# sourmash-bio/sourmash

Hardware: AMD Instinct MI355X
Metric: Gbase/s sketched (k=31, scaled=1000) (higher is better)
Workload: dtype u64; 1 GPU; C2: sketch synthetic random DNA resident in HBM as ASCII, per GPU 1000 records of 10000000 bases (10000000000 bases, 10000001000 bytes with their separators), k=31 scaled=1000 seed=42; one step = k-mer kernel + radix sort + unique; records_per_gpu=1000, record_len=10000000, bases_per_gpu=10000000000, bytes_per_gpu=10000001000, ksize=31, scaled=1000, unique_hashes_rank0=9998668, unique_hashes_job=9998668, collectives=none (the exchange runs with --full)

## Files before the change

include/sourmash_amd.h:

```cpp
#ifndef SOURMASH_AMD_H_INCLUDED
#define SOURMASH_AMD_H_INCLUDED

#include <stdarg.h>
#include <stdbool.h>
#include <stdint.h>
#include <stdlib.h>

#ifdef __cplusplus
extern "C" {
#endif


enum {
  HASH_FUNCTIONS_MURMUR64_DNA = 1,
  HASH_FUNCTIONS_MURMUR64_PROTEIN = 2,
  HASH_FUNCTIONS_MURMUR64_DAYHOFF = 3,
  HASH_FUNCTIONS_MURMUR64_HP = 4,
};
typedef uint32_t HashFunctions;

enum {
  SOURMASH_ERROR_CODE_NO_ERROR = 0,
  SOURMASH_ERROR_CODE_PANIC = 1,
  SOURMASH_ERROR_CODE_INTERNAL = 2,
// ... 196 lines not shown
uint64_t smgpu_minhash_pending_bytes(const SourmashKmerMinHash *ptr);
uint64_t smgpu_signature_add_file(SourmashSignature *ptr, const char *path, uint64_t *n_records);
SourmashSignature **smgpu_sketch_files(const char *const *paths, uintptr_t n, const SourmashComputeParameters *params,
                                       uint32_t n_threads, uint64_t *total_bases);
uint64_t smgpu_minhash_add_file(SourmashKmerMinHash *ptr, const char *path, uint64_t *n_records);
uint64_t smgpu_gunzip_files(const char *const *paths, uintptr_t n, uint8_t *out, uint64_t capacity, uint64_t *lens, double *stats);
void smgpu_sigload_counters(uint64_t *out);
void smgpu_gunzip_counters(uint64_t *out);

uint64_t smgpu_sketch_workspace_bytes(uint64_t out_capacity);
uint64_t smgpu_sketch_dna_raw(const uint8_t *d_seq, uint64_t len, uint32_t ksize, uint64_t seed, uint64_t max_hash,
                              uint64_t *d_out, uint64_t out_capacity, uint64_t *d_result, void *d_workspace,
                              uint64_t workspace_bytes, void *stream);
uint64_t smgpu_sketch_records_workspace_bytes(uint64_t pair_capacity, uint64_t n_records);
uint64_t smgpu_sketch_records_raw(const uint8_t *d_seq, uint64_t len, const uint64_t *d_starts, uint64_t n_records,
                                  uint32_t ksize, uint64_t seed, uint64_t max_hash, uint64_t *d_hashes, uint64_t *d_abunds,
                                  uint64_t capacity, uint64_t *d_offsets, uint64_t *d_result, void *d_workspace,
                                  uint64_t workspace_bytes, void *stream);
void smgpu_sketch_records_kernel_raw(const uint8_t *d_seq, uint64_t len, uint32_t ksize, uint64_t seed, uint64_t max_hash,
                                     uint64_t *d_hashes, uint64_t *d_positions, uint64_t capacity, uint64_t *d_count, void *stream);
void smgpu_fastx_compact_raw(const uint8_t *d_raw, uint64_t len, int32_t fastq, uint8_t *d_carry, uint8_t *d_out, uint64_t *d_result,
                             uint64_t *d_record_starts, uint64_t record_capacity, int32_t last_piece, void *stream);
uint64_t smgpu_sigjson_text_pad(void);
void smgpu_sigjson_parse_raw(const uint8_t *d_text, uint64_t text_len, const uint64_t *docs, uint32_t n_docs, uint64_t keep_max,
                             void *spans_out, uint32_t *flags_out, uint64_t *d_values, uint64_t value_capacity, void *parsed_out,
                             uint64_t parsed_capacity, uint64_t *counts_out, void *stream);
SourmashSignature **smgpu_sketch_file_singleton(const char *path, const SourmashComputeParameters *params, uintptr_t *n);
void smgpu_sketch_dna_kernel_raw(const uint8_t *d_seq, uint64_t len, uint32_t ksize, uint64_t seed, uint64_t max_hash,
                                 uint64_t *d_out, uint64_t out_capacity, uint64_t *d_count, void *stream);
void smgpu_sketch_dna_kernel_grid_raw(const uint8_t *d_seq, uint64_t len, uint32_t ksize, uint64_t seed, uint64_t max_hash,
                                      uint64_t *d_out, uint64_t out_capacity, uint64_t *d_count, uint32_t grid, void *stream);
uint64_t smgpu_sort_unique_raw(uint64_t *d_keys, uint64_t n, uint64_t *d_out, uint64_t *d_n_out, void *d_workspace,
                               uint64_t workspace_bytes, void *stream);
uint64_t smgpu_sketch_residues_kernels_raw(const uint8_t *d_seq, uint64_t len, uint32_t k_aa, uint32_t hash_function, uint64_t seed,
                                           uint64_t max_hash, bool translate, uint8_t *d_aa, uint64_t aa_capacity, uint64_t *d_out,
                                           uint64_t out_capacity, uint64_t *d_count, void *stream);
void smgpu_synth_dna_raw(uint8_t *d_out, uint64_t start, uint64_t n, uint64_t seed, uint64_t record_len, void *stream);

void smgpu_compare_raw(const uint64_t *d_hashes, const uint64_t *d_offsets, uint32_t n, uint32_t row_lo,
                       uint32_t row_hi, uint32_t *d_common, double *d_jaccard, void *stream);
void smgpu_compare_blocks_raw(const uint64_t *d_hashes, const uint64_t *d_offsets, uint32_t n, uint32_t rb_first,
                              uint32_t rb_stride, uint32_t rb_count, uint32_t *d_common, void *stream);
void smgpu_symmetrize_raw(uint32_t *d_common, uint32_t n, void *stream);
void smgpu_jaccard_raw(const uint32_t *d_common, const uint64_t *d_offsets, uint32_t n, uint32_t row_lo,
                       uint32_t row_hi, double *d_jaccard, void *stream);
typedef struct SmgpuBitIndex SmgpuBitIndex;
SmgpuBitIndex *smgpu_bitindex_new(const uint64_t *d_hashes, const uint64_t *d_offsets, uint32_t n, void *stream);
SmgpuBitIndex *smgpu_bitindex_new_ex(const uint64_t *d_hashes, const uint64_t *d_offsets, uint32_t n, uint64_t total_hashes,
                                     uint32_t threshold, bool one_shot, void *stream);
void smgpu_bitindex_free(SmgpuBitIndex *ptr);
uint64_t smgpu_bitindex_universe(const SmgpuBitIndex *ptr);
uint32_t smgpu_bitindex_builder(const SmgpuBitIndex *ptr);
void smgpu_bitindex_stats(const SmgpuBitIndex *ptr, uint64_t *frequent_hashes, uint64_t *rare_pairs, uint32_t *threshold);
void smgpu_bitindex_compare_raw(const SmgpuBitIndex *ptr, uint32_t rb_first, uint32_t rb_stride, uint32_t rb_count,
                                uint32_t *d_common, void *stream);
void smgpu_bitindex_compare_upper_raw(const SmgpuBitIndex *ptr, uint32_t rb_first, uint32_t rb_stride, uint32_t rb_count,
                                      uint32_t *d_common, void *stream);
void smgpu_host_pow_f64(const double *x, const double *y, uintptr_t ny, double *out, uintptr_t n, uint32_t n_threads);
uintptr_t smgpu_first_invalid_dna_byte(const char *seq, uintptr_t len);
void smgpu_compare_all_pairs(const SourmashKmerMinHash *const *mhs, uintptr_t n, uint32_t *common_out,
                             double *jaccard_out);
void smgpu_compare_all_pairs_mixed(const SourmashKmerMinHash *const *mhs, uintptr_t n, const uint32_t *class_of,
                                   const uint64_t *class_max_hash, uintptr_t n_classes, uint32_t *common_out, uint64_t *sizes_out);
void smgpu_signatures_sketch_views(const SourmashSignature *const *sigs, uintptr_t n, const SourmashKmerMinHash **out_mhs,
                                   uint64_t *params);
void smgpu_minhashes_params(const SourmashKmerMinHash *const *mhs, uintptr_t n, uint64_t *params);
// ... 148 lines not shown
```

sourmash_amd/csrc/capi.cpp:

```cpp
#if defined(__SSE2__)
#include <emmintrin.h>
#endif
#include <hip/hip_runtime_api.h>
#include <stdio.h>
#include <string.h>
#include <chrono>
#include <cmath>
#include <fstream>
#include <memory>
#include <sstream>
#include <thread>
#include "../../include/sourmash_amd.h"
#include "collection.hpp"
#include <fcntl.h>
#include <sys/mman.h>
#include <sys/stat.h>
#include <unistd.h>
#include "device_ctx.hpp"
#include "hostxfer.hpp"
#include "pargz.hpp"
#include "ingest.hpp"
#include "sigload.hpp"
#include "murmur3.hpp"
#include "residues.hpp"
#include "signature_host.hpp"
#include "hll_host.hpp"
#include "nodegraph_host.hpp"

using namespace smg;

namespace {

thread_local uint32_t g_err_code = 0;
thread_local std::string g_err_msg;

void set_error(uint32_t code, const std::string& msg) { g_err_code = code; g_err_msg = msg; }

template <class R, class F>
R landing(F&& f) {
    try {
        return f();
    } catch (const Error& e) {
        set_error(e.code, e.what());
    } catch (const std::bad_alloc&) {
        set_error(E_PANIC, "sourmash panicked: out of memory");
    } catch (const std::exception& e) {
        set_error(E_PANIC, std::string("sourmash panicked: ") + e.what());
    } catch (...) {
        set_error(E_PANIC, "sourmash panicked: unknown exception");
    }
    return R{};
}
template <class F>
void landing_void(F&& f) {
    landing<int>([&]() { f(); return 0; });
}
// ... 707 lines not shown
            lens[i] = ms[i].out_len;
            at += ms[i].out_len;
        }
        hip_check(hipStreamSynchronize(st), "sync");
        if (stats) {
            const double v[10] = {(double)gs.survivors, (double)gs.candidates, (double)gs.runs, gs.scan_ms, gs.pass1_ms, gs.link_ms, gs.pass2_ms,
                                  gs.finish_ms, gs.total_ms, io_ms};
            for (int k = 0; k < 16; ++k) stats[k] = k < 10 ? v[k] : 0.0;
        }
        return at;
    });
}
void smgpu_sigload_counters(uint64_t* out) {
    if (!out) return;
    out[0] = sigload_counters().on_device.load();
    out[1] = sigload_counters().on_host.load();
}
void smgpu_gunzip_counters(uint64_t* out) {
    if (!out) return;
    out[0] = gunzip_counters().on_device.load();
    out[1] = gunzip_counters().refused.load();
}
uint64_t smgpu_minhash_add_file(SourmashKmerMinHash* p, const char* path, uint64_t* n_records) {
    return landing<uint64_t>([&]() -> uint64_t {
        if (!path) throw err_internal("null path");
        std::vector<KmerMinHash*> mhs{MH(p)};
        uint64_t recs = 0, bases = 0;
        sketch_file_into(mhs, path, &recs, &bases);
        if (n_records) *n_records = recs;
        return bases;
    });
}

uint64_t smgpu_sketch_workspace_bytes(uint64_t out_capacity) {
    return (uint64_t)out_capacity * 8 + sort_unique_temp_bytes(out_capacity) + 512;
}

uint64_t smgpu_sketch_dna_raw(const uint8_t* d_seq, uint64_t len, uint32_t ksize, uint64_t seed, uint64_t max_hash,
                              uint64_t* d_out, uint64_t cap, uint64_t* d_result, void* d_ws, uint64_t ws_bytes,
                              void* stream) {
    uint64_t ret = ~0ull;
    landing_void([&] {
        hipStream_t st = (hipStream_t)stream;
        if (ws_bytes < smgpu_sketch_workspace_bytes(cap)) throw err_internal("workspace too small (smgpu_sketch_workspace_bytes)");
        uint64_t* d_raw = (uint64_t*)d_ws;
        void* d_tmp = (char*)d_ws + ((cap * 8 + 255) / 256) * 256;
        const size_t tmp_bytes = (size_t)(ws_bytes - ((cap * 8 + 255) / 256) * 256);
        const uint64_t thr = max_hash ? max_hash : ~0ull;
        check_dna_ksize(ksize);
        hip_check(hipMemsetAsync(d_result, 0, 16, st), "memset");
        hip_check(sketch_dna_launch(d_seq, len, ksize, seed, thr, d_raw, (unsigned long long*)d_result, cap, st), "sketch_dna");
        unsigned long long kept = 0;
        hip_check(hipMemcpyAsync(&kept, d_result, 8, hipMemcpyDeviceToHost, st), "D2H");
        hip_check(hipStreamSynchronize(st), "sync");
        if (kept > cap)
            throw err_internal("output capacity too small: " + std::to_string(kept) + " kept hashes > capacity " + std::to_string(cap));
        int bits = 64;
        if (thr != ~0ull) { bits = 1; while (bits < 64 && (thr >> bits)) ++bits; }
        hip_check(sort_unique(d_raw, kept, d_out, nullptr, d_result + 1, d_tmp, tmp_bytes, bits, st), "sort_unique");
        unsigned long long nu = 0;
        hip_check(hipMemcpyAsync(&nu, d_result + 1, 8, hipMemcpyDeviceToHost, st), "D2H");
        hip_check(hipStreamSynchronize(st), "sync");
        ret = nu;
    });
    return ret;
}

uint64_t smgpu_sort_unique_raw(uint64_t* d_keys, uint64_t n, uint64_t* d_out, uint64_t* d_n_out, void* d_ws, uint64_t ws_bytes, void* stream) {
    uint64_t ret = ~0ull;
    landing_void([&] {
        hipStream_t st = (hipStream_t)stream;
        if (ws_bytes < sort_unique_temp_bytes(n)) throw err_internal("workspace too small (smgpu_sketch_workspace_bytes)");
        hip_check(sort_unique(d_keys, n, d_out, nullptr, d_n_out, d_ws, (size_t)ws_bytes, 64, st), "sort_unique");
        unsigned long long nu = 0;
        hip_check(hipMemcpyAsync(&nu, d_n_out, 8, hipMemcpyDeviceToHost, st), "D2H");
        hip_check(hipStreamSynchronize(st), "sync");
        ret = nu;
    });
    return ret;
}

void smgpu_sketch_dna_kernel_raw(const uint8_t* d_seq, uint64_t len, uint32_t ksize, uint64_t seed, uint64_t max_hash,
                                 uint64_t* d_out, uint64_t cap, uint64_t* d_count, void* stream) {
    landing_void([&] {
        check_dna_ksize(ksize);
        hip_check(sketch_dna_launch(d_seq, len, ksize, seed, max_hash ? max_hash : ~0ull, d_out,
                                    (unsigned long long*)d_count, cap, (hipStream_t)stream), "sketch_dna");
    });
}
void smgpu_sketch_dna_kernel_grid_raw(const uint8_t* d_seq, uint64_t len, uint32_t ksize, uint64_t seed, uint64_t max_hash,
                                      uint64_t* d_out, uint64_t cap, uint64_t* d_count, uint32_t grid, void* stream) {
    landing_void([&] {
        check_dna_ksize(ksize);
        if (grid > (1u << 20)) throw err_internal("grid: at most 1048576 workgroups");
// ... 2460 lines not shown
```

sourmash_amd/csrc/device_api.hpp:

```cpp
#pragma once
#include <hip/hip_runtime.h>
#include <stdint.h>
#include <stddef.h>
#include "find_core.hpp"

namespace smg {

hipError_t sketch_dna_launch(const uint8_t* d_seq, uint64_t len, uint32_t k, uint64_t seed, uint64_t thr,
                             uint64_t* d_out, unsigned long long* d_count, uint64_t cap, hipStream_t stream);
hipError_t sketch_dna_launch_grid(const uint8_t* d_seq, uint64_t len, uint32_t k, uint64_t seed, uint64_t thr,
                                  uint64_t* d_out, unsigned long long* d_count, uint64_t cap, uint32_t grid, hipStream_t stream);
struct SketchMultiOut { uint64_t thr; uint64_t* out; unsigned long long* count; uint64_t cap; };
bool sketch_dna_multi_supported(const uint32_t* ks, int n);
hipError_t sketch_dna_multi_launch(const uint8_t* d_new, uint64_t n_new, const uint32_t* ks, int n, uint64_t seed, const SketchMultiOut* outs,
                                   hipStream_t stream);
hipError_t sketch_dna_words_launch(const uint8_t* d_seq, uint64_t len, uint32_t k, uint64_t seed, uint64_t thr, uint64_t* d_out,
                                   unsigned long long* d_count, uint64_t cap, bool dense, hipStream_t stream);
uint32_t sketch_dna_max_k();
hipError_t kmer_hashes_launch(const uint8_t* d_seq, uint64_t len, uint32_t k, uint64_t seed, uint64_t* d_out,
                              uint64_t n_kmers, hipStream_t stream);
hipError_t first_invalid_launch(const uint8_t* d_seq, uint64_t len, unsigned long long* d_first, hipStream_t stream);

hipError_t hll_dna_launch(const uint8_t* d_seq, uint64_t len, uint32_t k, uint32_t p, uint32_t* d_regs, hipStream_t stream);
hipError_t hll_hashes_launch(const uint64_t* d_hashes, uint64_t n, uint32_t p, uint32_t* d_regs, bool skip_zero, hipStream_t stream);
hipError_t hll_pack_launch(const uint32_t* d_regs, uint32_t n, uint8_t* d_out, hipStream_t stream);

struct NgTable { uint64_t size, magic, off; };
struct NgDev {
    const NgTable* tabs = nullptr;
    uint32_t n_tables = 0;
    uint32_t* words = nullptr;
    uint64_t n_words = 0;
    uint64_t t0_words = 0;
    unsigned long long* occ = nullptr;
};
hipError_t nodegraph_dna_launch(const uint8_t* d_seq, uint64_t len, uint32_t k, const NgDev& g, hipStream_t stream);
hipError_t nodegraph_hashes_launch(const uint64_t* d_hashes, uint64_t n, const NgDev& g, hipStream_t stream);
hipError_t nodegraph_matches_launch(const uint64_t* d_hashes, const uint64_t* d_offsets, uint64_t n_rows, const NgDev& g,
                                    uint64_t* d_out, hipStream_t stream);

hipError_t residues_launch(const uint8_t* d_seq, uint64_t len, uint32_t hash_function, uint8_t* d_aa, hipStream_t stream);
uint64_t translated_bytes(uint64_t len);
hipError_t translate_launch(const uint8_t* d_seq, uint64_t len, uint32_t hash_function, uint8_t* d_aa, hipStream_t stream);
hipError_t residue_windows_launch(const uint8_t* d_aa, uint64_t n, uint32_t k, uint64_t seed, uint64_t thr, uint64_t* d_out,
                                  unsigned long long* d_count, uint64_t cap, bool dense, hipStream_t stream);

size_t sort_unique_temp_bytes(uint64_t n);
struct TagSegment { uint64_t src, dst, n; };
hipError_t tag_gather_launch(const uint64_t* d_src, const TagSegment* d_segs, uint32_t n_segs, uint64_t* d_dst, int hbits, hipStream_t stream);
hipError_t sort_unique(uint64_t* d_keys, uint64_t n, uint64_t* d_out, uint64_t* d_counts, uint64_t* d_n_out,
                       void* d_temp, size_t temp_bytes, int bits, hipStream_t stream);

size_t sort_pairs_temp_bytes(uint64_t n);
hipError_t sort_pairs(const uint64_t* d_keys_in, uint64_t* d_keys_out, const uint64_t* d_vals_in, uint64_t* d_vals_out, uint64_t n,
                      int bits, void* d_temp, size_t temp_bytes, hipStream_t stream);
size_t rle_pairs_temp_bytes(uint64_t n);
hipError_t rle_pairs(const uint64_t* d_a, const uint64_t* d_b, uint64_t n, uint64_t* d_out_a, uint64_t* d_out_b, uint64_t* d_counts,
                     uint64_t* d_n_out, void* d_temp, size_t temp_bytes, hipStream_t stream);

hipError_t records_pairs_launch(const uint8_t* d_seq, uint64_t len, uint32_t k, uint64_t seed, uint64_t thr, uint64_t* d_hash,
                                uint64_t* d_pos, unsigned long long* d_count, uint64_t cap, hipStream_t stream);
hipError_t records_check_starts_launch(const uint64_t* d_starts, uint64_t n_records, uint64_t len, unsigned long long* d_bad,
                                       hipStream_t stream);
size_t records_csr_temp_bytes(uint64_t n_pairs);
hipError_t records_csr_launch(uint64_t* d_pair_hash, uint64_t* d_pair_pos, uint64_t n_pairs, const uint64_t* d_starts, uint64_t n_records,
                              uint32_t k, uint64_t max_hash, uint64_t* d_hashes, uint64_t* d_abunds, uint64_t* d_offsets, uint64_t* d_n_out,
                              void* d_temp, size_t temp_bytes, hipStream_t stream);

hipError_t find_dir_launch(const uint64_t* d_q, uint64_t n, uint32_t shift, uint64_t n_buckets, uint32_t* d_dir, hipStream_t stream);
hipError_t find_pairs_launch(const uint8_t* d_seq, uint64_t len, uint32_t k, uint64_t seed, const FindQuery& query, uint64_t* d_hash,
                             uint64_t* d_pos, unsigned long long* d_count, uint64_t cap, uint32_t grid, hipStream_t stream);
size_t find_rows_temp_bytes(uint64_t n_pairs);
hipError_t find_rows_launch(const uint8_t* d_seq, uint64_t len, uint64_t* d_pair_hash, uint64_t* d_pair_pos, uint64_t n_pairs,
                            const uint64_t* d_starts, uint64_t n_records, uint32_t k, uint64_t* d_positions, uint64_t* d_hashes,
                            uint8_t* d_kmers, uint64_t* d_offsets, uint64_t* d_n_out, void* d_temp, size_t temp_bytes, hipStream_t stream);

hipError_t synth_dna_launch(uint8_t* d_out, uint64_t start, uint64_t n, uint64_t seed, uint64_t record_len,
                            hipStream_t stream);

hipError_t compare_counts_launch(const uint64_t* d_hashes, const uint64_t* d_offsets, uint32_t n,
                                 uint32_t row_lo, uint32_t row_hi, uint32_t* d_common ,
                                 hipStream_t stream);
hipError_t compare_blocks_launch(const uint64_t* d_hashes, const uint64_t* d_offsets, uint32_t n, uint32_t rb_first,
                                 uint32_t rb_stride, uint32_t rb_count, uint32_t* d_common, hipStream_t stream);
// ... 46 lines not shown
```

sourmash_amd/device.py:

```python
import ctypes as C

from ._lowlevel import lib
from .minhash import _get_max_hash_for_scaled
from .exceptions import SourmashError, exceptions_by_code
from .utils import decode_str, rustcall


def _torch():
    import torch
    if not torch.cuda.is_available():
        raise RuntimeError("sourmash_amd.device needs a HIP device (no CPU fallback)")
    return torch


def _ptr(t):
    return C.c_void_p(t.data_ptr())


def _stream(torch):
    return C.c_void_p(torch.cuda.current_stream().cuda_stream)


def _u64(torch, n, device):
    return torch.empty(int(n), dtype=torch.int64, device=device)
# ... 130 lines not shown
            if code == 0:
                return (hashes[:got], offsets, abunds[:got]) if abund else (hashes[:got], offsets)
            message = decode_str(lib.sourmash_err_get_last_message())
            kept = int(result[0].item())
            if attempt == 0 and kept > cap:
                cap = kept
                continue
            raise _records_error(code, message)

    def records_kernel_only(self, seq, out_hashes, out_positions, count):
        torch = self.torch
        rustcall(lib.smgpu_sketch_records_kernel_raw, _ptr(seq), seq.numel(), self.ksize, self.seed, self.max_hash,
                 _ptr(out_hashes), _ptr(out_positions), min(out_hashes.numel(), out_positions.numel()), _ptr(count), _stream(torch))

    def kernel_only(self, seq, out, count, grid=0):
        torch = self.torch
        rustcall(lib.smgpu_sketch_dna_kernel_grid_raw, _ptr(seq), seq.numel(), self.ksize, self.seed, self.max_hash,
                 _ptr(out), out.numel(), _ptr(count), int(grid), _stream(torch))


def sort_unique(keys):
    torch = _torch()
    assert keys.dtype == torch.int64 and keys.is_cuda and keys.is_contiguous()
    n = keys.numel()
    out = _u64(torch, max(n, 1), keys.device)
    if n == 0:
        return out[:0]
    ws = torch.empty(int(lib.smgpu_sketch_workspace_bytes(n)), dtype=torch.uint8, device=keys.device)
    n_out = torch.zeros(1, dtype=torch.int64, device=keys.device)
    m = rustcall(lib.smgpu_sort_unique_raw, _ptr(keys), n, _ptr(out), _ptr(n_out), _ptr(ws), ws.numel(), _stream(torch))
    return out[:m]


def pack_csr(sketches, device="cuda"):
    import numpy as np
    torch = _torch()
    offsets = np.zeros(len(sketches) + 1, dtype=np.int64)
    for i, s in enumerate(sketches):
        offsets[i + 1] = offsets[i] + len(s)
    flat = np.concatenate([np.asarray(s, dtype=np.uint64) for s in sketches]) if len(sketches) and offsets[-1] \
        else np.zeros(0, dtype=np.uint64)
    hashes = torch.from_numpy(flat.view(np.int64).copy()).to(device)
    if hashes.numel() == 0:
        hashes = torch.zeros(2, dtype=torch.int64, device=device)
    return hashes, torch.from_numpy(offsets).to(device)


class BitIndex:

    def __init__(self, ptr, n):
        self._ptr, self.n = ptr, n

    @classmethod
    def build(cls, hashes, offsets, threshold=None, one_shot=False):
        torch = _torch()
        n = offsets.numel() - 1
        ptr = rustcall(lib.smgpu_bitindex_new_ex, _ptr(hashes), _ptr(offsets), n, 0, int(threshold or 0), bool(one_shot),
                       _stream(torch))
        return cls(ptr, n) if ptr else None

    @property
    def universe(self):
        return lib.smgpu_bitindex_universe(self._ptr)

    @property
    def builder(self):
# ... 50 lines not shown
```

Baseline: 370.3 Gbase/s.

## Replace radix sort with uniform-key bucket sort and unique for sketch hashes

Adds a bucket-based sort+unique that exploits the uniform distribution of hash values below max_hash: one or two scatter passes distribute keys into fixed-capacity leaves, per-leaf LDS sort and dedup, then a scan and pack. This avoids the multi-pass radix sort and also removes the host sync that read the kept count before sorting, since the device-side count drives the kernels. If a leaf overflows, a flag triggers a fallback to the old radix path, which adds an extra sync and redundant work in that case.

```diff
diff --git a/include/sourmash_amd.h b/include/sourmash_amd.h
--- a/include/sourmash_amd.h
+++ b/include/sourmash_amd.h
@@ -252,6 +252,11 @@
                                       uint64_t *d_out, uint64_t out_capacity, uint64_t *d_count, uint32_t grid, void *stream);
 uint64_t smgpu_sort_unique_raw(uint64_t *d_keys, uint64_t n, uint64_t *d_out, uint64_t *d_n_out, void *d_workspace,
                                uint64_t workspace_bytes, void *stream);
+uint64_t smgpu_sort_unique_uniform_workspace_bytes(uint64_t n_max, int32_t counts);
+uint64_t smgpu_sort_unique_uniform_raw(uint64_t *d_keys, const uint64_t *d_n, uint64_t n_max, uint64_t thr, uint64_t *d_out,
+                                       uint64_t *d_counts, uint64_t *d_result, void *d_workspace, uint64_t workspace_bytes,
+                                       void *stream);
+void smgpu_sort_counters(uint64_t *out);
 uint64_t smgpu_sketch_residues_kernels_raw(const uint8_t *d_seq, uint64_t len, uint32_t k_aa, uint32_t hash_function, uint64_t seed,
                                            uint64_t max_hash, bool translate, uint8_t *d_aa, uint64_t aa_capacity, uint64_t *d_out,
                                            uint64_t out_capacity, uint64_t *d_count, void *stream);
diff --git a/sourmash_amd/csrc/capi.cpp b/sourmash_amd/csrc/capi.cpp
--- a/sourmash_amd/csrc/capi.cpp
+++ b/sourmash_amd/csrc/capi.cpp
@@ -4,6 +4,8 @@
 #include <hip/hip_runtime_api.h>
 #include <stdio.h>
 #include <string.h>
+#include <algorithm>
+#include <atomic>
 #include <chrono>
 #include <cmath>
 #include <fstream>
@@ -22,6 +24,7 @@
 #include "ingest.hpp"
 #include "sigload.hpp"
 #include "murmur3.hpp"
+#include "uniform_sort_core.hpp"
 #include "residues.hpp"
 #include "signature_host.hpp"
 #include "hll_host.hpp"
@@ -795,8 +798,42 @@
     });
 }
 
+static size_t sketch_ws_raw_bytes(uint64_t cap) { return (size_t)((cap * 8 + 255) / 256) * 256; }
+static size_t sketch_ws_sort_bytes(uint64_t cap, bool counts) {
+    return std::max(sort_unique_temp_bytes(cap), sort_unique_uniform_temp_bound(cap, counts));
+}
 uint64_t smgpu_sketch_workspace_bytes(uint64_t out_capacity) {
-    return (uint64_t)out_capacity * 8 + sort_unique_temp_bytes(out_capacity) + 512;
+    return (uint64_t)sketch_ws_raw_bytes(out_capacity) + 256 + sketch_ws_sort_bytes(out_capacity, false) + 512;
+}
+
+struct SortCounters { std::atomic<uint64_t> bucket{0}, small{0}, fellback{0}; };
+static SortCounters& sort_counters() { static SortCounters c; return c; }
+void smgpu_sort_counters(uint64_t* out) {
+    if (!out) return;
+    out[0] = sort_counters().bucket.load();
+    out[1] = sort_counters().small.load();
+    out[2] = sort_counters().fellback.load();
+}
+
+static void uniform_sort_and_report(const uint64_t* d_keys, const unsigned long long* d_n, uint64_t n_max, uint64_t thr, uint64_t* d_out,
+                                    uint64_t* d_counts, uint64_t* d_n_out, void* d_head, void* d_tmp, size_t tmp_bytes, hipStream_t st,
+                                    uint64_t report[3]) {
+    uint64_t* d_report = (uint64_t*)d_head;
+    uint32_t* d_flag = (uint32_t*)((char*)d_head + 64);
+    hip_check(sort_unique_uniform(d_keys, d_n, n_max, thr, d_out, d_counts, d_n_out, d_flag, d_tmp, tmp_bytes, st), "sort_unique_uniform");
+    hip_check(sort_report_launch(d_n, d_n_out, d_flag, d_report, st), "sort_report");
+    hip_check(hipMemcpyAsync(report, d_report, 24, hipMemcpyDeviceToHost, st), "D2H");
+    hip_check(hipStreamSynchronize(st), "sync");
+}
+static void count_sort_call(uint64_t n_max, uint64_t thr, size_t tmp_bytes, bool counts, bool fellback) {
+    if (fellback) ++sort_counters().fellback;
+    else if (sort_unique_uniform_form(n_max, thr, tmp_bytes, counts) == US_SMALL) ++sort_counters().small;
+    else ++sort_counters().bucket;
+}
+static int key_bits(uint64_t thr) {
+    int bits = 64;
+    if (thr != ~0ull) { bits = 1; while (bits < 64 && (thr >> bits)) ++bits; }
+    return bits;
 }
 
 uint64_t smgpu_sketch_dna_raw(const uint8_t* d_seq, uint64_t len, uint32_t ksize, uint64_t seed, uint64_t max_hash,
@@ -807,22 +844,52 @@
         hipStream_t st = (hipStream_t)stream;
         if (ws_bytes < smgpu_sketch_workspace_bytes(cap)) throw err_internal("workspace too small (smgpu_sketch_workspace_bytes)");
         uint64_t* d_raw = (uint64_t*)d_ws;
-        void* d_tmp = (char*)d_ws + ((cap * 8 + 255) / 256) * 256;
-        const size_t tmp_bytes = (size_t)(ws_bytes - ((cap * 8 + 255) / 256) * 256);
+        void* d_head = (char*)d_ws + sketch_ws_raw_bytes(cap);
+        void* d_tmp = (char*)d_head + 256;
+        const size_t tmp_bytes = (size_t)(ws_bytes - sketch_ws_raw_bytes(cap) - 256);
         const uint64_t thr = max_hash ? max_hash : ~0ull;
         check_dna_ksize(ksize);
         hip_check(hipMemsetAsync(d_result, 0, 16, st), "memset");
         hip_check(sketch_dna_launch(d_seq, len, ksize, seed, thr, d_raw, (unsigned long long*)d_result, cap, st), "sketch_dna");
-        unsigned long long kept = 0;
-        hip_check(hipMemcpyAsync(&kept, d_result, 8, hipMemcpyDeviceToHost, st), "D2H");
-        hip_check(hipStreamSynchronize(st), "sync");
+        uint64_t report[3] = {0, 0, 0};
+        uniform_sort_and_report(d_raw, (const unsigned long long*)d_result, cap, thr, d_out, nullptr, d_result + 1, d_head, d_tmp, tmp_bytes,
+                                st, report);
+        const uint64_t kept = report[0];
         if (kept > cap)
             throw err_internal("output capacity too small: " + std::to_string(kept) + " kept hashes > capacity " + std::to_string(cap));
-        int bits = 64;
-        if (thr != ~0ull) { bits = 1; while (bits < 64 && (thr >> bits)) ++bits; }
-        hip_check(sort_unique(d_raw, kept, d_out, nullptr, d_result + 1, d_tmp, tmp_bytes, bits, st), "sort_unique");
+        count_sort_call(cap, thr, tmp_bytes, false, report[2] != 0);
+        if (report[2] == 0) { ret = report[1]; return; }
+        hip_check(sort_unique(d_raw, kept, d_out, nullptr, d_result + 1, d_tmp, tmp_bytes, key_bits(thr), st), "sort_unique");
         unsigned long long nu = 0;
         hip_check(hipMemcpyAsync(&nu, d_result + 1, 8, hipMemcpyDeviceToHost, st), "D2H");
+        hip_check(hipStreamSynchronize(st), "sync");
+        ret = nu;
+    });
+    return ret;
+}
+
+uint64_t smgpu_sort_unique_uniform_workspace_bytes(uint64_t n_max, int32_t counts) {
+    return 256 + (uint64_t)sketch_ws_sort_bytes(n_max, counts != 0) + 512;
+}
+
+uint64_t smgpu_sort_unique_uniform_raw(uint64_t* d_keys, const uint64_t* d_n, uint64_t n_max, uint64_t thr, uint64_t* d_out, uint64_t* d_counts,
+                                       uint64_t* d_result, void* d_ws, uint64_t ws_bytes, void* stream) {
+    uint64_t ret = ~0ull;
+    landing_void([&] {
+        hipStream_t st = (hipStream_t)stream;
+        if (!d_keys || !d_n || !d_out || !d_result || !d_ws) throw err_internal("null pointer");
+        if (ws_bytes < smgpu_sort_unique_uniform_workspace_bytes(n_max, d_counts != nullptr))
+            throw err_internal("workspace too small (smgpu_sort_unique_uniform_workspace_bytes)");
+        void* d_tmp = (char*)d_ws + 256;
+        const size_t tmp_bytes = (size_t)(ws_bytes - 256);
+        uint64_t report[3] = {0, 0, 0};
+        uniform_sort_and_report(d_keys, (const unsigned long long*)d_n, n_max, thr, d_out, d_counts, d_result, d_ws, d_tmp, tmp_bytes, st, report);
+        count_sort_call(n_max, thr, tmp_bytes, d_counts != nullptr, report[2] != 0);
+        if (report[2] == 0) { ret = report[1]; return; }
+        const uint64_t n = std::min(report[0], n_max);
+        hip_check(sort_unique(d_keys, n, d_out, d_counts, d_result, d_tmp, tmp_bytes, 64, st), "sort_unique");
+        unsigned long long nu = 0;
+        hip_check(hipMemcpyAsync(&nu, d_result, 8, hipMemcpyDeviceToHost, st), "D2H");
         hip_check(hipStreamSynchronize(st), "sync");
         ret = nu;
     });
diff --git a/sourmash_amd/csrc/device_api.hpp b/sourmash_amd/csrc/device_api.hpp
--- a/sourmash_amd/csrc/device_api.hpp
+++ b/sourmash_amd/csrc/device_api.hpp
@@ -50,6 +50,15 @@
 hipError_t tag_gather_launch(const uint64_t* d_src, const TagSegment* d_segs, uint32_t n_segs, uint64_t* d_dst, int hbits, hipStream_t stream);
 hipError_t sort_unique(uint64_t* d_keys, uint64_t n, uint64_t* d_out, uint64_t* d_counts, uint64_t* d_n_out,
                        void* d_temp, size_t temp_bytes, int bits, hipStream_t stream);
+
+hipError_t sort_unique_uniform(const uint64_t* d_keys, const unsigned long long* d_n, uint64_t n_max, uint64_t thr, uint64_t* d_out,
+                               uint64_t* d_counts, uint64_t* d_n_out, uint32_t* d_fellback, void* d_temp, size_t temp_bytes,
+                               hipStream_t stream);
+size_t sort_unique_uniform_temp_bytes(uint64_t n_max, uint64_t thr, bool counts);
+size_t sort_unique_uniform_temp_bound(uint64_t n_max, bool counts);
+uint32_t sort_unique_uniform_form(uint64_t n_max, uint64_t thr, size_t temp_bytes, bool counts);
+hipError_t sort_report_launch(const unsigned long long* d_n, const uint64_t* d_n_out, const uint32_t* d_fellback, uint64_t* d_report,
+                              hipStream_t stream);
 
 size_t sort_pairs_temp_bytes(uint64_t n);
 hipError_t sort_pairs(const uint64_t* d_keys_in, uint64_t* d_keys_out, const uint64_t* d_vals_in, uint64_t* d_vals_out, uint64_t n,
diff --git a/sourmash_amd/csrc/uniform_sort.hip b/sourmash_amd/csrc/uniform_sort.hip
--- /dev/null
+++ b/sourmash_amd/csrc/uniform_sort.hip
@@ -0,0 +1,388 @@
+#include <hip/hip_runtime.h>
+#include "device_api.hpp"
+#include "uniform_sort_core.hpp"
+
+namespace smg {
+namespace {
+
+constexpr uint32_t NO_BASE = 0xffffffffu;
+
+__device__ __forceinline__ uint64_t us_count(const unsigned long long* d_n, uint64_t n_max) {
+    const uint64_t n = *d_n;
+    return n < n_max ? n : n_max;
+}
+
+template <int T>
+__device__ __forceinline__ void us_sort_lds(uint64_t* keys, uint32_t n) {
+    const uint32_t P = us_pow2(n);
+    for (uint32_t k = 2, j = 0; k <= P; us_next_step(k, j)) {
+        for (uint32_t t = threadIdx.x; t < P / 2; t += T) {
+            uint32_t a, b;
+            us_pair(t, k, j, a, b);
+            us_compare_exchange(keys, n, a, b);
+        }
+        __syncthreads();
+    }
+}
+
+template <int T>
+__device__ __forceinline__ uint32_t us_block_scan(uint32_t v, uint32_t* wsum, uint32_t& total) {
+    const uint32_t lane = threadIdx.x & 63, wave = threadIdx.x >> 6;
+    uint32_t x = v;
+#pragma unroll
+    for (uint32_t off = 1; off < 64; off <<= 1) {
+        const uint32_t y = __shfl_up(x, off);
+        if (lane >= off) x += y;
+    }
+    if (lane == 63) wsum[wave] = x;
+    __syncthreads();
+    uint32_t base = 0, all = 0;
+#pragma unroll
+    for (uint32_t w = 0; w < T / 64; ++w) {
+        const uint32_t t = wsum[w];
+        if (w < wave) base += t;
+        all += t;
+    }
+    __syncthreads();
+    total = all;
+    return base + x - v;
+}
+
+template <int T, int E, int B, bool LEAF>
+__device__ __forceinline__ void us_sort_keys(const uint64_t* src, uint32_t n, uint32_t bin_shift, uint64_t* s, uint32_t* bins,
+                                             uint32_t* wsum) {
+    constexpr int BPT = B / T;
+    static_assert(B % T == 0, "bins per thread");
+#pragma unroll
+    for (int i = 0; i < BPT; ++i) bins[threadIdx.x + i * T] = 0;
+    __syncthreads();
+    uint64_t key[E];
+    uint32_t at[E];
+#pragma unroll
+    for (int e = 0; e < E; ++e) {
+        const uint32_t i = threadIdx.x + e * T;
+        key[e] = 0;
+        at[e] = 0;
+        if (i < n) {
+            key[e] = src[i];
+            at[e] = atomicAdd(&bins[LEAF ? us_bin_leaf(bin_shift, key[e]) : us_bin_small(bin_shift, key[e])], 1u);
+        }
+    }
+    __syncthreads();
+    uint32_t mine[BPT], sum = 0, most = 0;
+#pragma unroll
+    for (int i = 0; i < BPT; ++i) {
+        mine[i] = bins[threadIdx.x * BPT + i];
+        sum += mine[i];
+        most = mine[i] > most ? mine[i] : most;
+    }
+    uint32_t total;
+    uint32_t start = us_block_scan<T>(sum, wsum, total);
+    if (__syncthreads_or(most > US_BIN_LIMIT)) {
+#pragma unroll
+        for (int e = 0; e < E; ++e)
+            if (threadIdx.x + e * T < n) s[threadIdx.x + e * T] = key[e];
+        __syncthreads();
+        us_sort_lds<T>(s, n);
+        return;
+    }
+#pragma unroll
+    for (int i = 0; i < BPT; ++i) {
+        bins[threadIdx.x * BPT + i] = start;
+        start += mine[i];
+    }
+    if (threadIdx.x == T - 1) bins[B] = start;
+    __syncthreads();
+#pragma unroll
+    for (int e = 0; e < E; ++e) {
+        if (threadIdx.x + e * T >= n) continue;
+        at[e] += bins[LEAF ? us_bin_leaf(bin_shift, key[e]) : us_bin_small(bin_shift, key[e])];
+        s[at[e]] = key[e];
+    }
+    __syncthreads();
+#pragma unroll
+    for (int e = 0; e < E; ++e) {
+        if (threadIdx.x + e * T >= n) continue;
+        const uint32_t b = LEAF ? us_bin_leaf(bin_shift, key[e]) : us_bin_small(bin_shift, key[e]);
+        const uint32_t lo = bins[b], hi = bins[b + 1];
+        uint32_t rank = lo;
+        for (uint32_t m = lo; m < hi; ++m) rank += us_before(s[m], m, key[e], at[e]) ? 1u : 0u;
+        at[e] = rank;
+    }
+    __syncthreads();
+#pragma unroll
+    for (int e = 0; e < E; ++e)
+        if (threadIdx.x + e * T < n) s[at[e]] = key[e];
+    __syncthreads();
+}
+
+template <int T, int E, typename CT>
+__device__ __forceinline__ uint32_t us_unique_write(const uint64_t* keys, uint32_t n, uint32_t* scan, uint64_t* out, CT* counts) {
+    const uint32_t lo = threadIdx.x * E;
+    uint32_t heads = 0;
+#pragma unroll
+    for (int e = 0; e < E; ++e)
+        if (lo + e < n && us_is_head(keys, lo + e)) ++heads;
+    uint32_t total;
+    const uint32_t first = us_block_scan<T>(heads, scan, total);
+    uint32_t q = first;
+#pragma unroll
+    for (int e = 0; e < E; ++e) {
+        const uint32_t i = lo + e;
+        if (i < n && us_is_head(keys, i)) {
+            out[q] = keys[i];
+            if (counts) counts[q] = (CT)0 - (CT)i;
+            ++q;
+        }
+    }
+    if (counts) {
+        __syncthreads();
+        q = first;
+#pragma unroll
+        for (int e = 0; e < E; ++e) {
+            const uint32_t i = lo + e;
+            if (i >= n) break;
+            if (us_is_head(keys, i)) ++q;
+            if (us_is_tail(keys, n, i)) counts[q - 1] += (CT)(i + 1);
+        }
+    }
+    return total;
+}
+
+__global__ __launch_bounds__(1024) void us_small_kernel(const uint64_t* __restrict__ keys, const unsigned long long* __restrict__ d_n,
+                                                        uint64_t n_max, uint32_t small_shift, uint64_t* __restrict__ out,
+                                                        uint64_t* __restrict__ counts, uint64_t* __restrict__ d_n_out,
+                                                        uint32_t* __restrict__ d_fellback) {
+    __shared__ uint64_t s[US_SMALL_MAX];
+    __shared__ uint32_t bins[US_SMALL_BINS + 1];
+    __shared__ uint32_t scan[1024 / 64];
+    const uint32_t n = (uint32_t)us_count(d_n, n_max < US_SMALL_MAX ? n_max : US_SMALL_MAX);
+    us_sort_keys<1024, US_SMALL_MAX / 1024, US_SMALL_BINS, false>(keys, n, small_shift, s, bins, scan);
+    const uint32_t total = us_unique_write<1024, US_SMALL_MAX / 1024, uint64_t>(s, n, scan, out, counts);
+    if (threadIdx.x == 0) {
+        *d_n_out = total;
+        *d_fellback = 0;
+    }
+}
+
+template <bool SECOND>
+__global__ __launch_bounds__(256) void us_scatter_kernel(const UsPlan p, const uint64_t* __restrict__ src,
+                                                         const unsigned long long* __restrict__ d_n, uint64_t n_max,
+                                                         const uint32_t* __restrict__ src_cursor, uint32_t tiles_per_region,
+                                                         uint32_t* __restrict__ cursor, uint64_t* __restrict__ dst, uint64_t dst_cap,
+                                                         uint32_t* __restrict__ d_fellback) {
+    __shared__ uint32_t hist[US_FANOUT];
+    __shared__ uint32_t base[US_FANOUT];
+    uint64_t region = 0, begin, n;
+    if (!SECOND) {
+        n = us_count(d_n, n_max);
+        begin = (uint64_t)blockIdx.x * US_TILE;
+    } else {
+        __shared__ uint32_t quit;
+        if (threadIdx.x == 0) quit = *d_fellback;
+        __syncthreads();
+        if (quit) return;
+        region = blockIdx.x / tiles_per_region;
+        const uint64_t held = src_cursor[region];
+        n = held < p.region_cap ? held : p.region_cap;
+        begin = (uint64_t)(blockIdx.x % tiles_per_region) * US_TILE;
+        src += region * p.region_cap;
+        cursor += region * US_FANOUT;
+        dst += region * US_FANOUT * dst_cap;
+    }
+    if (begin >= n) return;
+    hist[threadIdx.x] = 0;
+    __syncthreads();
+    constexpr int E = US_TILE / 256;
+    uint64_t key[E];
+    uint32_t digit[E], rank[E];
+    bool stray = false;
+#pragma unroll
+    for (int e = 0; e < E; ++e) {
+        const uint64_t i = begin + (uint64_t)e * 256 + threadIdx.x;
+        digit[e] = US_FANOUT;
+        rank[e] = 0;
+        key[e] = 0;
+        if (i < n) {
+            key[e] = src[i];
+            digit[e] = SECOND ? us_digit_second(p, region, key[e]) : us_digit_first(p, key[e]);
+            if (digit[e] < US_FANOUT) rank[e] = atomicAdd(&hist[digit[e]], 1u);
+            else stray = true;
+        }
+    }
+    if (stray) atomicOr(d_fellback, 1u);
+    __syncthreads();
+    {
+        const uint32_t c = hist[threadIdx.x];
+        uint32_t b = NO_BASE;
+        if (c) {
+            const uint32_t at = atomicAdd(&cursor[threadIdx.x], c);
+            if (us_reserve_ok(at, c, dst_cap)) b = at;
+            else atomicOr(d_fellback, 1u);
+        }
+        base[threadIdx.x] = b;
+    }
+    __syncthreads();
+#pragma unroll
+    for (int e = 0; e < E; ++e) {
+        if (digit[e] >= US_FANOUT) continue;
+        const uint32_t b = base[digit[e]];
+        if (b != NO_BASE) dst[(uint64_t)digit[e] * dst_cap + b + rank[e]] = key[e];
+    }
+}
+
+__global__ __launch_bounds__(256) void us_leaf_kernel(uint32_t shift, const uint32_t* __restrict__ cursor, uint64_t* __restrict__ leaves,
+                                                      uint32_t* __restrict__ leaf_counts, uint32_t* __restrict__ leaf_distinct,
+                                                      const uint32_t* __restrict__ d_fellback) {
+    __shared__ uint64_t s[US_LEAF_CAP];
+    __shared__ uint32_t bins[US_LEAF_BINS + 1];
+    __shared__ uint32_t scan[256 / 64];
+    if (*d_fellback) return;
+    const uint64_t leaf = blockIdx.x;
+    const uint32_t held = cursor[leaf];
+    const uint32_t n = held < US_LEAF_CAP ? held : US_LEAF_CAP;
+    uint64_t* mine = leaves + leaf * US_LEAF_CAP;
+    us_sort_keys<256, US_LEAF_CAP / 256, US_LEAF_BINS, true>(mine, n, shift, s, bins, scan);
+    const uint32_t total = us_unique_write<256, US_LEAF_CAP / 256, uint32_t>(s, n, scan, mine,
+                                                                            leaf_counts ? leaf_counts + leaf * US_LEAF_CAP : nullptr);
+    if (threadIdx.x == 0) leaf_distinct[leaf] = total;
+}
+
+__global__ __launch_bounds__(1024) void us_scan_kernel(const uint32_t* __restrict__ leaf_distinct, uint32_t n_leaves,
+                                                       uint32_t* __restrict__ offsets, uint64_t* __restrict__ d_n_out,
+                                                       const uint32_t* __restrict__ d_fellback) {
+    __shared__ uint32_t wsum[1024 / 64];
+    if (*d_fellback) return;
+    uint32_t carry = 0;
+    for (uint32_t base = 0; base < n_leaves; base += 4096) {
+        const uint32_t l = base + threadIdx.x * 4;
+        uint32_t v[4], sum = 0, total;
+#pragma unroll
+        for (int i = 0; i < 4; ++i) {
+            v[i] = l + i < n_leaves ? leaf_distinct[l + i] : 0;
+            sum += v[i];
+        }
+        uint32_t at = carry + us_block_scan<1024>(sum, wsum, total);
+#pragma unroll
+        for (int i = 0; i < 4; ++i) {
+            if (l + i < n_leaves) offsets[l + i] = at;
+            at += v[i];
+        }
+        carry += total;
+    }
+    if (threadIdx.x == 0) {
+        offsets[n_leaves] = carry;
+        *d_n_out = carry;
+    }
+}
+
+__global__ __launch_bounds__(256) void us_pack_kernel(const uint64_t* __restrict__ leaves, const uint32_t* __restrict__ leaf_counts,
+                                                      const uint32_t* __restrict__ offsets, uint64_t* __restrict__ out,
+                                                      uint64_t* __restrict__ counts, const uint32_t* __restrict__ d_fellback) {
+    if (*d_fellback) return;
+    const uint64_t leaf = blockIdx.x;
+    const uint32_t at = offsets[leaf], n = offsets[leaf + 1] - at;
+    for (uint32_t i = threadIdx.x; i < n; i += 256) {
+        out[at + i] = leaves[leaf * US_LEAF_CAP + i];
+        if (counts) counts[at + i] = leaf_counts[leaf * US_LEAF_CAP + i];
+    }
+}
+
+__global__ void us_report_kernel(const unsigned long long* __restrict__ d_n, const uint64_t* __restrict__ d_n_out,
+                                 const uint32_t* __restrict__ d_fellback, uint64_t* __restrict__ report) {
+    report[0] = *d_n;
+    report[1] = *d_n_out;
+    report[2] = *d_fellback;
+}
+
+size_t up256(size_t x) { return (x + 255) / 256 * 256; }
+
+struct UsLayout {
+    size_t coarse_cursors, leaf_cursors, cursor_bytes, distinct, offsets, coarse, leaves, counts, total;
+};
+UsLayout us_layout(const UsPlan& p, bool counts) {
+    UsLayout y{};
+    const size_t n_leaf_cursors = p.form == US_TWO_PASS ? (size_t)p.regions * US_FANOUT : US_FANOUT;
+    y.coarse_cursors = 0;
+    y.leaf_cursors = up256(US_FANOUT * 4);
+    y.cursor_bytes = y.leaf_cursors + up256(n_leaf_cursors * 4);
+    y.distinct = y.cursor_bytes;
+    y.offsets = y.distinct + up256(n_leaf_cursors * 4);
+    y.coarse = y.offsets + up256((n_leaf_cursors + 1) * 4);
+    y.leaves = y.coarse + up256((size_t)p.regions * p.region_cap * 8);
+    y.counts = y.leaves + up256((size_t)p.leaves * US_LEAF_CAP * 8);
+    y.total = y.counts + (counts ? up256((size_t)p.leaves * US_LEAF_CAP * 4) : 0);
+    return y;
+}
+
+}
+
+size_t sort_unique_uniform_temp_bytes(uint64_t n_max, uint64_t thr, bool counts) {
+    const UsPlan p = us_plan(n_max, thr);
+    if (p.form == US_SMALL || p.form == US_DECLINE) return 256;
+    return us_layout(p, counts).total;
+}
+
+size_t sort_unique_uniform_temp_bound(uint64_t n_max, bool counts) {
+    if (n_max <= US_SMALL_MAX) return 256;
+    return up256((size_t)n_max * 8 * 5 + (counts ? (size_t)n_max * 4 * 3 : 0) + ((size_t)8 << 20));
+}
+
+uint32_t sort_unique_uniform_form(uint64_t n_max, uint64_t thr, size_t temp_bytes, bool counts) {
+    const UsPlan p = us_plan(n_max, thr);
+    if (p.form == US_SMALL || p.form == US_DECLINE) return p.form;
+    return temp_bytes < us_layout(p, counts).total ? (uint32_t)US_DECLINE : p.form;
+}
+
+hipError_t sort_unique_uniform(const uint64_t* d_keys, const unsigned long long* d_n, uint64_t n_max, uint64_t thr, uint64_t* d_out,
+                               uint64_t* d_counts, uint64_t* d_n_out, uint32_t* d_fellback, void* d_temp, size_t temp_bytes,
+                               hipStream_t stream) {
+    const UsPlan p = us_plan(n_max, thr);
+    const uint32_t form = sort_unique_uniform_form(n_max, thr, temp_bytes, d_counts != nullptr);
+    if (form == US_SMALL) {
+        hipLaunchKernelGGL(us_small_kernel, dim3(1), dim3(1024), 0, stream, d_keys, d_n, n_max, us_small_shift(thr), d_out, d_counts, d_n_out,
+                           d_fellback);
+        return hipGetLastError();
+    }
+    if (form == US_DECLINE) return hipMemsetD32Async((hipDeviceptr_t)d_fellback, 1, 1, stream);
+    const UsLayout y = us_layout(p, d_counts != nullptr);
+    char* base = (char*)d_temp;
+    uint32_t* coarse_cursors = (uint32_t*)(base + y.coarse_cursors);
+    uint32_t* leaf_cursors = (uint32_t*)(base + y.leaf_cursors);
+    uint32_t* distinct = (uint32_t*)(base + y.distinct);
+    uint32_t* offsets = (uint32_t*)(base + y.offsets);
+    uint64_t* coarse = (uint64_t*)(base + y.coarse);
+    uint64_t* leaves = (uint64_t*)(base + y.leaves);
+    uint32_t* leaf_counts = d_counts ? (uint32_t*)(base + y.counts) : nullptr;
+    hipError_t e = hipMemsetAsync(d_fellback, 0, 4, stream);
+    if (e != hipSuccess) return e;
+    e = hipMemsetAsync(base, 0, y.cursor_bytes, stream);
+    if (e != hipSuccess) return e;
+    const uint32_t tiles = (uint32_t)((n_max + US_TILE - 1) / US_TILE);
+    if (form == US_ONE_PASS) {
+        hipLaunchKernelGGL(us_scatter_kernel<false>, dim3(tiles), dim3(256), 0, stream, p, d_keys, d_n, n_max, (const uint32_t*)nullptr, 1u,
+                           leaf_cursors, leaves, (uint64_t)US_LEAF_CAP, d_fellback);
+    } else {
+        hipLaunchKernelGGL(us_scatter_kernel<false>, dim3(tiles), dim3(256), 0, stream, p, d_keys, d_n, n_max, (const uint32_t*)nullptr, 1u,
+                           coarse_cursors, coarse, p.region_cap, d_fellback);
+        const uint32_t tpr = (uint32_t)((p.region_cap + US_TILE - 1) / US_TILE);
+        hipLaunchKernelGGL(us_scatter_kernel<true>, dim3((uint32_t)p.regions * tpr), dim3(256), 0, stream, p, (const uint64_t*)coarse, d_n,
+                           n_max, (const uint32_t*)coarse_cursors, tpr, leaf_cursors, leaves, (uint64_t)US_LEAF_CAP, d_fellback);
+    }
+    const uint32_t L = (uint32_t)p.leaves;
+    hipLaunchKernelGGL(us_leaf_kernel, dim3(L), dim3(256), 0, stream, p.shift, (const uint32_t*)leaf_cursors, leaves, leaf_counts, distinct,
+                       (const uint32_t*)d_fellback);
+    hipLaunchKernelGGL(us_scan_kernel, dim3(1), dim3(1024), 0, stream, (const uint32_t*)distinct, L, offsets, d_n_out,
+                       (const uint32_t*)d_fellback);
+    hipLaunchKernelGGL(us_pack_kernel, dim3(L), dim3(256), 0, stream, (const uint64_t*)leaves, (const uint32_t*)leaf_counts,
+                       (const uint32_t*)offsets, d_out, d_counts, (const uint32_t*)d_fellback);
+    return hipGetLastError();
+}
+
+hipError_t sort_report_launch(const unsigned long long* d_n, const uint64_t* d_n_out, const uint32_t* d_fellback, uint64_t* d_report,
+                              hipStream_t stream) {
+    hipLaunchKernelGGL(us_report_kernel, dim3(1), dim3(1), 0, stream, d_n, d_n_out, d_fellback, d_report);
+    return hipGetLastError();
+}
+
+}
diff --git a/sourmash_amd/csrc/uniform_sort_core.hpp b/sourmash_amd/csrc/uniform_sort_core.hpp
--- /dev/null
+++ b/sourmash_amd/csrc/uniform_sort_core.hpp
@@ -0,0 +1,121 @@
+#pragma once
+#include <stdint.h>
+
+#if defined(__HIPCC__)
+#include <hip/hip_runtime.h>
+#endif
+
+#ifndef SMG_HD
+#if defined(__HIPCC__)
+#define SMG_HD __host__ __device__ __forceinline__
+#else
+#define SMG_HD inline
+#endif
+#endif
+
+namespace smg {
+
+constexpr uint32_t US_SMALL_MAX = 16384;
+constexpr uint32_t US_LEAF_CAP = 1024;
+constexpr uint32_t US_FANOUT = 256;
+constexpr uint32_t US_TILE = 4096;
+constexpr uint64_t US_MAX_LEAVES = (uint64_t)US_FANOUT * US_FANOUT;
+
+enum UsForm : uint32_t { US_DECLINE = 0, US_SMALL = 1, US_ONE_PASS = 2, US_TWO_PASS = 3 };
+
+struct UsPlan {
+    uint32_t form;
+    uint32_t shift;
+    uint64_t leaves;
+    uint64_t regions;
+    uint64_t region_cap;
+    uint64_t thr;
+};
+
+SMG_HD uint64_t us_isqrt_up(uint64_t x) {
+    uint64_t r = 0;
+    while (r * r < x) ++r;
+    return r;
+}
+
+SMG_HD bool us_load_fits(uint64_t load, uint64_t cap) {
+    if (load >= cap) return false;
+    const uint64_t spare = cap - load;
+    return spare * spare >= 64 * load;
+}
+
+SMG_HD uint64_t us_leaves(uint64_t thr, uint32_t shift) { return (thr >> shift) + 1; }
+
+SMG_HD UsPlan us_plan(uint64_t n_max, uint64_t thr) {
+    UsPlan p{US_DECLINE, 0, 0, 0, 0, thr};
+    if (n_max <= US_SMALL_MAX) { p.form = US_SMALL; return p; }
+    if (n_max > 0xffffffffull) return p;
+    int shift = 63;
+    for (; shift >= 0; --shift) {
+        const uint64_t L = us_leaves(thr, (uint32_t)shift);
+        if (L > US_MAX_LEAVES) return p;
+        if (us_load_fits((n_max + L - 1) / L, US_LEAF_CAP)) break;
+    }
+    if (shift < 0) return p;
+    p.shift = (uint32_t)shift;
+    p.leaves = us_leaves(thr, p.shift);
+    if (p.leaves <= US_FANOUT) { p.form = US_ONE_PASS; return p; }
+    p.form = US_TWO_PASS;
+    p.regions = ((p.leaves - 1) >> 8) + 1;
+    const uint64_t load = ((n_max + p.leaves - 1) / p.leaves) * US_FANOUT;
+    p.region_cap = load + 8 * us_isqrt_up(load);
+    return p;
+}
+
+SMG_HD uint64_t us_leaf_of(const UsPlan& p, uint64_t key) { return key >> p.shift; }
+SMG_HD uint32_t us_digit_first(const UsPlan& p, uint64_t key) {
+    if (key > p.thr) return US_FANOUT;
+    const uint64_t leaf = us_leaf_of(p, key);
+    return (uint32_t)(p.form == US_TWO_PASS ? leaf >> 8 : leaf);
+}
+SMG_HD uint32_t us_digit_second(const UsPlan& p, uint64_t region, uint64_t key) {
+    if (key > p.thr) return US_FANOUT;
+    const uint64_t leaf = us_leaf_of(p, key);
+    return (leaf >> 8) == region ? (uint32_t)(leaf & 0xff) : US_FANOUT;
+}
+SMG_HD bool us_reserve_ok(uint64_t base, uint64_t count, uint64_t cap) { return base <= cap && count <= cap - base; }
+
+constexpr uint32_t US_LEAF_BINS = 1024;
+constexpr uint32_t US_SMALL_BINS = 4096;
+constexpr uint32_t US_BIN_LIMIT = 32;
+SMG_HD uint32_t us_bin_leaf(uint32_t shift, uint64_t key) { return (uint32_t)(key >> (shift > 10 ? shift - 10 : 0)) & (US_LEAF_BINS - 1); }
+SMG_HD uint32_t us_small_shift(uint64_t thr) {
+    uint32_t s = 0;
+    while (s < 63 && (thr >> s) >= US_SMALL_BINS) ++s;
+    return s;
+}
+SMG_HD uint32_t us_bin_small(uint32_t small_shift, uint64_t key) {
+    const uint64_t b = key >> small_shift;
+    return b < US_SMALL_BINS ? (uint32_t)b : US_SMALL_BINS - 1;
+}
+SMG_HD bool us_before(uint64_t other, uint32_t other_at, uint64_t key, uint32_t at) { return other < key || (other == key && other_at < at); }
+
+SMG_HD uint32_t us_pow2(uint32_t n) {
+    uint32_t p = 1;
+    while (p < n) p <<= 1;
+    return p;
+}
+SMG_HD void us_pair(uint32_t t, uint32_t k, uint32_t j, uint32_t& a, uint32_t& b) {
+    const uint32_t off = t & ((j == 0 ? k >> 1 : j) - 1);
+    a = 2 * (t - off) + off;
+    b = j == 0 ? 2 * (t - off) + k - 1 - off : a + j;
+}
+SMG_HD void us_compare_exchange(uint64_t* keys, uint32_t n, uint32_t a, uint32_t b) {
+    if (b >= n) return;
+    const uint64_t x = keys[a], y = keys[b];
+    if (x > y) { keys[a] = y; keys[b] = x; }
+}
+SMG_HD void us_next_step(uint32_t& k, uint32_t& j) {
+    if (j == 0) j = k >> 2; else j >>= 1;
+    if (j == 0) k <<= 1;
+}
+
+SMG_HD bool us_is_head(const uint64_t* keys, uint32_t i) { return i == 0 || keys[i] != keys[i - 1]; }
+SMG_HD bool us_is_tail(const uint64_t* keys, uint32_t n, uint32_t i) { return i + 1 == n || keys[i] != keys[i + 1]; }
+
+}
diff --git a/sourmash_amd/device.py b/sourmash_amd/device.py
--- a/sourmash_amd/device.py
+++ b/sourmash_amd/device.py
@@ -186,6 +186,28 @@
     return out[:m]
 
 
+def sort_unique_uniform(keys, max_hash, n=None, counts=False):
+    torch = _torch()
+    assert keys.dtype == torch.int64 and keys.is_cuda and keys.is_contiguous()
+    n_max = keys.numel()
+    out = _u64(torch, max(n_max, 1), keys.device)
+    cnt = _u64(torch, max(n_max, 1), keys.device) if counts else None
+    d_n = torch.tensor([n_max if n is None else int(n)], dtype=torch.int64, device=keys.device)
+    result = torch.zeros(1, dtype=torch.int64, device=keys.device)
+    ws = torch.empty(int(lib.smgpu_sort_unique_uniform_workspace_bytes(n_max, int(counts))), dtype=torch.uint8, device=keys.device)
+    thr = int(max_hash) if max_hash else 0xFFFFFFFFFFFFFFFF
+    m = rustcall(lib.smgpu_sort_unique_uniform_raw, _ptr(keys) if n_max else _ptr(out), _ptr(d_n), n_max, thr, _ptr(out),
+                 _ptr(cnt) if counts else None, _ptr(result), _ptr(ws), ws.numel(), _stream(torch))
+    return (out[:m], cnt[:m]) if counts else out[:m]
+
+
+def sort_counters():
+    import ctypes
+    out = (ctypes.c_uint64 * 3)()
+    lib.smgpu_sort_counters(out)
+    return {"bucket": int(out[0]), "small": int(out[1]), "fellback": int(out[2])}
+
+
 def pack_csr(sketches, device="cuda"):
     import numpy as np
     torch = _torch()
```

Result: faster. 375.2 Gbase/s, median of 6 (+1.3%).
